# CPJKU/audio_sheet_retrieval

Hardware: AMD Instinct MI355X
Metric: snippet-pairs/sec embedded+ranked (32-d CCA) (higher is better)
Workload: dtype f32

## Files before the change

### audio_sheet_retrieval_amd/csrc/conv_wino_kernels.hip

```cpp
#include <hip/hip_runtime.h>
#include <stdint.h>
#include <stdlib.h>
#include <algorithm>
#include <type_traits>
#include <vector>
#include "asr_kernels.h"
#include "repack_elems.inl"
#include "wino_tile_order.h"
#include "wino_weight_layout.h"

#ifndef ASR_WINOG_NOCOPY
#define ASR_WINOG_NOCOPY 1
#endif

#ifndef ASR_WINOG_ABL
#define ASR_WINOG_ABL 0
#endif

namespace asr {

typedef float floatx4w __attribute__((ext_vector_type(4)));
typedef float float2w __attribute__((ext_vector_type(2)));

#ifndef ASR_WINO_ASMREAD
#define ASR_WINO_ASMREAD 1
#endif
#ifndef ASR_WINO_BUFDMA
#define ASR_WINO_BUFDMA 1
#endif

struct WinoArgs {
    const float *in;
    const float *wpk;
    const float *bnp;
    float *out;
    int N, H, W, OH, OW;
    int RY, RX;
    int MY, MX;
    int nmy, nmx;
    int tiles_y, tiles_x;
    int coutp;
    int C4P, RP;
    int total;
    int per;
    double *stats;
    BnBwdFuse bf;
    const void *raw;
    const float *w1;
    const float *bn1;
};

#ifndef ASR_WINO_PKADD
#define ASR_WINO_PKADD 1
#endif
__device__ __forceinline__ float ssub(float a, float b) {
    float r;
    asm("v_sub_f32 %0, %1, %2" : "=v"(r) : "v"(a), "v"(b));
    return r;
}
__device__ __forceinline__ float2w psub(float2w a, float2w b) {
    if (ASR_WINO_PKADD) return a - b;
    return float2w{ssub(a[0], b[0]), ssub(a[1], b[1])};
}
__device__ __forceinline__ floatx4w psub(floatx4w a, floatx4w b) {
    if (ASR_WINO_PKADD) return a - b;
    return floatx4w{ssub(a[0], b[0]), ssub(a[1], b[1]), ssub(a[2], b[2]), ssub(a[3], b[3])};
}
__device__ __forceinline__ float sadd(float a, float b) {
    float r;
    asm("v_add_f32 %0, %1, %2" : "=v"(r) : "v"(a), "v"(b));
    return r;
}
__device__ __forceinline__ float2w padd(float2w a, float2w b) {
    if (ASR_WINO_PKADD) return a + b;
    return float2w{sadd(a[0], b[0]), sadd(a[1], b[1])};
}
__device__ __forceinline__ floatx4w padd(floatx4w a, floatx4w b) {
    if (ASR_WINO_PKADD) return a + b;
    return floatx4w{sadd(a[0], b[0]), sadd(a[1], b[1]), sadd(a[2], b[2]), sadd(a[3], b[3])};
}

__device__ float4 g_wino_zero[4];

template <int NTV>
__device__ __forceinline__ void wino_stats_store(double *stats, int row, int cout, int col0, int lane,
                                                 const double (&s1)[NTV], const double (&s2)[NTV]) {
    const int g = lane >> 4, n = lane & 15;
#pragma unroll
    for (int nt = 0; nt < NTV; ++nt) {
        double a = s1[nt], b = s2[nt];
        a += __shfl_xor(a, 16); b += __shfl_xor(b, 16);
        a += __shfl_xor(a, 32); b += __shfl_xor(b, 32);
        const int ch = col0 + nt * 16 + n;
        if (g == 0 && ch < cout) {
            stats[((size_t)row * 2) * cout + ch] = a;
            stats[((size_t)row * 2 + 1) * cout + ch] = b;
        }
    }
}

__device__ __forceinline__ float elu_fastw(float y) { return y > 0.0f ? y : __expf(y) - 1.0f; }

template <int CIN, int COUT, bool POOL, int NTW, int KB, int WAVES, int MINW, int RMAX, bool RAW, int PW = 0,
          int IN_MODE = 0>
__global__ __launch_bounds__(64 * (WAVES + PW), MINW) void conv3x3_wino(WinoArgs a) {
    constexpr int KS = CIN / 4;
    constexpr int NB = CIN / 8;
    constexpr bool REM = (CIN % 8) != 0;
    constexpr int NCH = NB / KB;
    constexpr int WROW = NTW * 16;
    constexpr int WS = NTW == 2 ? 48 : WROW;
    constexpr int C4 = CIN / 4;
    constexpr int T = 64 * (WAVES + PW);
    static_assert(NB % KB == 0, "chunking must divide the channel blocks");
    static_assert(PW == 0 || (!RAW && NTW * 16 >= COUT), "producer builds: deterministic path, one n-group");
    extern __shared__ __align__(16) float lds[];
    const int tid = threadIdx.x, lane = tid & 63;
    const int wave = __builtin_amdgcn_readfirstlane(tid >> 6);
    const int LW = a.RX + 2, LH = a.RY + 2;
    constexpr int C4P = (C4 & 1) ? C4 : C4 + 1;
    constexpr int CSf = C4P * 4;
    const int RPf = a.RP * 4;
    const int buf_floats = (LH * RPf + 255) & ~255;
    float *w_lds = lds + 2 * buf_floats;
    const int ng = blockIdx.y;
    const int first = blockIdx.x * a.per;
    const int last = min(first + a.per, a.total);
    if (first >= last) return;

    for (int i = tid; i < 16 * KS * 4 * (WROW / 4); i += T) {
        const int row = i / (WROW / 4), q = i - row * (WROW / 4);
        const int col = ng * WROW + q * 4;
        float4 v = make_float4(0.f, 0.f, 0.f, 0.f);
        if (col < a.coutp) v = *reinterpret_cast<const float4 *>(a.wpk + (size_t)row * a.coutp + col);
        *reinterpret_cast<float4 *>(w_lds + row * WS + q * 4) = v;
    }
    constexpr int RMAXE = PW > 0 ? 1 : RMAX;
    int st_g[RMAXE], st_rc[RMAXE];
    if constexpr (PW == 0) {
#pragma unroll
        for (int k = 0; k < RMAX; ++k) {
            const int f = tid + k * T;
            const int r = f / a.RP;
            const int xs = f - r * a.RP - ((r >> 1) & 1);
            const int px = xs / C4P, c = xs - px * C4P;
            const bool real = r < LH && xs >= 0 && px < LW && c < C4;
#if ASR_WINO_BUFDMA
            st_g[k] = real ? (((r - 1) * a.W + (px - 1)) * CIN + c * 4) * 4 : (int)0x80000000;
#else
            st_g[k] = ((r - 1) * a.W + (px - 1)) * CIN + c * 4;
#endif
            st_rc[k] = real ? (r << 16) | px : -1;
        }
    }
    auto fetch = [&](int region, float *buf) {
        if constexpr (PW == 0) {
        const int tx = region % a.tiles_x;
        const int rest = region / a.tiles_x;
        const int ty = rest % a.tiles_y;
        const int img = rest / a.tiles_y;
        const int Y0 = ty * a.RY, X0 = tx * a.RX;
#if ASR_WINO_BUFDMA
        {
            typedef int int4v __attribute__((ext_vector_type(4)));
            const uint64_t ibase = reinterpret_cast<uint64_t>(a.in + (int64_t)img * a.H * a.W * CIN);
            int4v rsrc;
            rsrc.x = (int)(uint32_t)ibase;
            rsrc.y = (int)(uint32_t)(ibase >> 32);
            rsrc.z = a.H * a.W * CIN * 4;
            rsrc.w = 0x00020000;
            const int roff = (Y0 * a.W + X0) * CIN * 4;
            const unsigned lds0 = (unsigned)(uintptr_t)(__attribute__((address_space(3))) void *)buf;
            const bool xedge = X0 < 1 || X0 + LW - 1 > a.W;
            auto dma = [&](int k, int vo) {
                const unsigned m0v = lds0 + (unsigned)((k * T + wave * 64) * 16);
                asm volatile("s_mov_b32 m0, %2\n\ts_nop 0\n\tbuffer_load_dwordx4 %0, %1, 0 offen lds"
                             ::"v"(vo), "s"(rsrc), "s"(m0v)
                             : "memory", "m0");
            };
            if (!__builtin_amdgcn_readfirstlane((int)xedge)) {
#pragma unroll
                for (int k = 0; k < RMAX; ++k) {
                    if ((k * T + wave * 64) * 4 >= buf_floats) break;
                    dma(k, st_g[k] + roff);
                }
                return;
            }
#pragma unroll
            for (int k = 0; k < RMAX; ++k) {
                if ((k * T + wave * 64) * 4 >= buf_floats) break;
                const int x = X0 - 1 + (st_rc[k] & 0xffff);
                dma(k, (st_rc[k] >= 0 && (unsigned)x < (unsigned)a.W) ? st_g[k] + roff : (int)0x80000000);
            }
            return;
        }
#endif
        const float *gbase = a.in + (((int64_t)img * a.H + Y0) * a.W + X0) * CIN;
        if (!(ASR_WINOG_ABL & 512) && Y0 >= 1 && Y0 + LH - 1 <= a.H && X0 >= 1 && X0 + LW - 1 <= a.W) {
#pragma unroll
            for (int k = 0; k < RMAX; ++k) {
                if ((k * T + wave * 64) * 4 >= buf_floats) break;
                const float *src = st_rc[k] >= 0 ? gbase + st_g[k] : reinterpret_cast<const float *>(g_wino_zero);
                __builtin_amdgcn_global_load_lds((const __attribute__((address_space(1))) void *)src,
                                                 (__attribute__((address_space(3))) void *)(buf + (k * T + wave * 64) * 4),
                                                 16, 0, 0);
            }
            return;
        }
#pragma unroll
        for (int k = 0; k < RMAX; ++k) {
            if ((k * T + wave * 64) * 4 >= buf_floats) break;
            const int y = Y0 - 1 + (st_rc[k] >> 16), x = X0 - 1 + (st_rc[k] & 0xffff);
            const bool ok = st_rc[k] >= 0 && y >= 0 && y < a.H && x >= 0 && x < a.W;
            const float *src = ok ? gbase + st_g[k] : reinterpret_cast<const float *>(g_wino_zero);
            __builtin_amdgcn_global_load_lds((const __attribute__((address_space(1))) void *)src,
                                             (__attribute__((address_space(3))) void *)(buf + (k * T + wave * 64) * 4),
                                             16, 0, 0);
        }
        }
    };
    float *tab255 = w_lds + 16 * KS * 4 * WS;
    auto produce = [&](int region, float *buf) {
        if constexpr (PW > 0) {
        const int ptid = tid - 64 * WAVES;
        const int tx = region % a.tiles_x;
        const int rest = region / a.tiles_x;
        const int ty = rest % a.tiles_y;
        const int img = rest / a.tiles_y;
        const int Y0 = ty * a.RY, X0 = tx * a.RX;
        const size_t ioff = (size_t)img * a.H * a.W;
        const int npx = LH * LW;
        const float rcpLW = 1.0f / (float)LW;
        for (int f = ptid; f < npx; f += 64 * PW) {
            const int r = (int)(((float)f + 0.5f) * rcpLW), px = f - r * LW;
            const int y = Y0 - 1 + r, x = X0 - 1 + px;
            float *dst = buf + (r * a.RP + ((r >> 1) & 1) + px * C4P) * 4;
            if (y < 0 || y >= a.H || x < 0 || x >= a.W) {
#pragma unroll
                for (int c = 0; c < C4; ++c) *reinterpret_cast<float4 *>(dst + c * 4) = make_float4(0.f, 0.f, 0.f, 0.f);
                continue;
            }
            float v[9];
#pragma unroll
            for (int aa = 0; aa < 3; ++aa)
#pragma unroll
                for (int bb = 0; bb < 3; ++bb) {
                    const int yy = y - 1 + aa, xx = x - 1 + bb;
                    const bool ok = yy >= 0 && yy < a.H && xx >= 0 && xx < a.W;
                    const int yc = min(max(yy, 0), a.H - 1), xc = min(max(xx, 0), a.W - 1);
                    const size_t off = ioff + (size_t)yc * a.W + xc;
                    float val;
                    if (IN_MODE == 2) val = tab255[((const unsigned char *)a.raw)[off]];
                    else if (IN_MODE == 1) val = ((const float *)a.raw)[off] / 255.0f;
                    else val = ((const float *)a.raw)[off];
                    v[aa * 3 + bb] = ok ? val : 0.0f;
                }
            constexpr int C1P = (CIN + 15) / 16 * 16;
#pragma unroll 1
            for (int cg = 0; cg < C4; ++cg) {
                const float *wg = a.w1 + cg * 36;
                float res[4];
#pragma unroll
                for (int c = 0; c < 4; ++c) {
                    const int co = cg * 4 + c;
                    float acc = 0.0f;
#pragma unroll
                    for (int t = 0; t < 9; ++t) acc = fmaf(v[t], wg[c * 9 + t], acc);
                    res[c] = elu_fastw((acc - a.bn1[co]) * a.bn1[C1P + co] + a.bn1[2 * C1P + co]);
                }
                *reinterpret_cast<float4 *>(dst + cg * 4) = make_float4(res[0], res[1], res[2], res[3]);
            }
        }
        }
    };
    const bool producer = PW > 0 && wave >= WAVES;
    if constexpr (PW > 0) {
        if (IN_MODE == 2)
            for (int i = tid; i < 256; i += T) tab255[i] = (float)i / 255.0f;
        __syncthreads();
        if (producer) produce(first, lds);
    } else {
        fetch(first, lds);
#if ASR_WINO_BUFDMA
        asm volatile("s_waitcnt vmcnt(0)" ::: "memory");
#endif
    }
    __syncthreads();

    const int m = lane & 15, g = lane >> 4, n = lane & 15;
    const int tyy = m / a.MX, txx = m - tyy * a.MX;
    int a_row[4];
#pragma unroll
    for (int i = 0; i < 4; ++i)
        a_row[i] = (2 * tyy + i) * RPf + 2 * txx * CSf + ((tyy + (i >> 1)) & 1) * 4;
    const int a_pair = (g >> 1) * 4 + (g & 1) * 2;
    const int a_rem = NB * 8 + g;
    const float *w_lane = w_lds + g * WS + n;
    auto wq_off = [](int q) { return ((q / (16 * NTW)) * 16 + (q / NTW) % 16) * 4 * WS + (q % NTW) * 16; };
    int ey[4], ex[4], eoff[4];
#pragma unroll
    for (int r = 0; r < 4; ++r) {
        const int me = 4 * g + r;
        ey[r] = me / a.MX;
        ex[r] = me - ey[r] * a.MX;
        eoff[r] = (POOL ? ey[r] * a.OW + ex[r] : 2 * ey[r] * a.W + 2 * ex[r]) * COUT + ng * WROW + n;
    }
    float bmean[NTW], bscale[NTW], bbeta[NTW];
#pragma unroll
    for (int nt = 0; nt < NTW; ++nt) {
        const int ch = ng * WROW + nt * 16 + n;
        const bool ok = !RAW && ch < COUT;
        bmean[nt] = ok ? a.bnp[ch] : 0.f;
        bscale[nt] = ok ? a.bnp[a.coutp + ch] : 1.f;
        bbeta[nt] = ok ? a.bnp[2 * a.coutp + ch] : 0.f;
    }
    float bistd[NTW];
    const bool bnb = ASR_BNB_FUSE_BUILD && RAW && a.stats && a.bf.z != nullptr;
#pragma unroll
    for (int nt = 0; nt < NTW; ++nt) {
        const int ch = ng * WROW + nt * 16 + n;
        bistd[nt] = 0.f;
        if (bnb && ch < COUT) {
            bmean[nt] = a.bf.cst[ch]; bistd[nt] = a.bf.cst[COUT + ch];
            bscale[nt] = a.bf.cst[2 * COUT + ch]; bbeta[nt] = a.bf.cst[3 * COUT + ch];
        }
    }

    double st1[NTW], st2[NTW];
#pragma unroll
    for (int nt = 0; nt < NTW; ++nt) { st1[nt] = 0.0; st2[nt] = 0.0; }
    for (int region = first; region < last; ++region) {
    const float *in_lds = lds + ((region - first) & 1) * buf_floats;
    if (region + 1 < last && !(ASR_WINOG_ABL & 1)) {
        if constexpr (PW > 0) {
            if (producer) produce(region + 1, lds + ((region + 1 - first) & 1) * buf_floats);
        } else {
            fetch(region + 1, lds + ((region + 1 - first) & 1) * buf_floats);
        }
    }
    const int tx = region % a.tiles_x;
    const int rest = region / a.tiles_x;
    const int ty = rest % a.tiles_y;
    const int img = rest / a.tiles_y;
    const int Y0 = ty * a.RY, X0 = tx * a.RX;
    for (int mt = producer ? a.nmy * a.nmx : wave; mt < a.nmy * a.nmx; mt += WAVES) {
        const int mty = mt / a.nmx, mtx = mt - mty * a.nmx;
        const int oy = mty * a.MY * 2, ox = mtx * a.MX * 2;
        if (Y0 + oy >= a.H || X0 + ox >= a.W) continue;
        const float *ap = in_lds + oy * RPf + ox * CSf;
        floatx4w acc[16][NTW];
#pragma unroll
        for (int p = 0; p < 16; ++p)
#pragma unroll
            for (int nt = 0; nt < NTW; ++nt) acc[p][nt] = floatx4w{0.f, 0.f, 0.f, 0.f};

#pragma unroll
        for (int ch = 0; ch < NCH + (REM ? 1 : 0); ++ch) {
            if (ch < NCH) {
                float2w dp[4][4][KB];
#if ASR_WINO_ASMREAD
                if (ASR_WINOG_ABL & 32) {
#pragma unroll
                    for (int i = 0; i < 4; ++i)
#pragma unroll
                        for (int j = 0; j < 4; ++j)
#pragma unroll
                            for (int c = 0; c < KB; ++c) dp[i][j][c] = float2w{(float)i, (float)j};
                } else {
#pragma unroll
                    for (int i = 0; i < 4; ++i) {
                        const unsigned la = (unsigned)(uintptr_t)(const __attribute__((address_space(3))) void *)(ap + a_row[i] + a_pair);
#pragma unroll
                        for (int j = 0; j < 4; ++j)
#pragma unroll
                            for (int c = 0; c < KB; ++c)
                                asm volatile("ds_read_b64 %0, %1 offset:%2"
                                             : "=v"(dp[i][j][c])
                                             : "v"(la), "n"((j * CSf + (ch * KB + c) * 8) * 4));
                    }
#pragma unroll
                    for (int c = 0; c < KB; ++c)
                        asm volatile("s_waitcnt lgkmcnt(0)"
                                     : "+v"(dp[0][0][c]), "+v"(dp[0][1][c]), "+v"(dp[0][2][c]), "+v"(dp[0][3][c]),
                                       "+v"(dp[1][0][c]), "+v"(dp[1][1][c]), "+v"(dp[1][2][c]), "+v"(dp[1][3][c]),
                                       "+v"(dp[2][0][c]), "+v"(dp[2][1][c]), "+v"(dp[2][2][c]), "+v"(dp[2][3][c]),
                                       "+v"(dp[3][0][c]), "+v"(dp[3][1][c]), "+v"(dp[3][2][c]), "+v"(dp[3][3][c]));
                }
#else
#pragma unroll
                for (int i = 0; i < 4; ++i)
#pragma unroll
                    for (int j = 0; j < 4; ++j)
#pragma unroll
                        for (int c = 0; c < KB; ++c)
                            dp[i][j][c] = (ASR_WINOG_ABL & 32) ? float2w{(float)i, (float)j}
                                                               : *reinterpret_cast<const float2w *>(ap + a_row[i] + j * CSf + (ch * KB + c) * 8 + a_pair);
#endif
#pragma unroll
                for (int c = 0; c < KB; ++c) {
#pragma unroll
                    for (int j = 0; j < 4; ++j) {
                        const float2w d0 = dp[0][j][c], d1 = dp[1][j][c], d2 = dp[2][j][c], d3 = dp[3][j][c];
                        dp[0][j][c] = psub(d0, d2); dp[1][j][c] = padd(d1, d2); dp[2][j][c] = psub(d2, d1); dp[3][j][c] = psub(d1, d3);
                    }
#pragma unroll
                    for (int i = 0; i < 4; ++i) {
                        const float2w t0 = dp[i][0][c], t1 = dp[i][1][c], t2 = dp[i][2][c], t3 = dp[i][3][c];
                        dp[i][0][c] = psub(t0, t2); dp[i][1][c] = padd(t1, t2); dp[i][2][c] = psub(t2, t1); dp[i][3][c] = psub(t1, t3);
                    }
                }
                constexpr int WQ = 2 * KB * 16 * NTW, WD = 4 * NTW;
                const float *wk = w_lane + (ch * 2 * KB) * (16 * 4 * WS);
                float wv[WQ + WD];
#pragma unroll
                for (int q = 0; q < WD; ++q) wv[q] = wk[wq_off(q)];
#pragma unroll
                for (int q0 = 0; q0 < WQ; q0 += NTW) {
#pragma unroll
                    for (int q = q0; q < q0 + NTW; ++q)
                        wv[q + WD] = (ASR_WINOG_ABL & 16) ? wv[q] : (q + WD < WQ) ? wk[wq_off(q + WD)] : 0.f;
                    __builtin_amdgcn_sched_barrier(0);
#pragma unroll
                    for (int q = q0; q < q0 + NTW; ++q) {
                        const int p = (q / NTW) % 16, c = q / (16 * NTW), nt = q % NTW;
                        acc[p][nt] = __builtin_amdgcn_mfma_f32_16x16x4f32(dp[p >> 2][p & 3][c >> 1][c & 1], wv[q],
                                                                          acc[p][nt], 0, 0, 0);
                    }
                    __builtin_amdgcn_sched_barrier(0);
                }
            } else {
                float dsg[4][4];
#pragma unroll
                for (int i = 0; i < 4; ++i)
#pragma unroll
                    for (int j = 0; j < 4; ++j) dsg[i][j] = (ASR_WINOG_ABL & 32) ? (float)(i + j) : ap[a_row[i] + j * CSf + a_rem];
#pragma unroll
                for (int j = 0; j < 4; ++j) {
                    const float d0 = dsg[0][j], d1 = dsg[1][j], d2 = dsg[2][j], d3 = dsg[3][j];
                    dsg[0][j] = d0 - d2; dsg[1][j] = d1 + d2; dsg[2][j] = d2 - d1; dsg[3][j] = d1 - d3;
                }
#pragma unroll
                for (int i = 0; i < 4; ++i) {
                    const float t0 = dsg[i][0], t1 = dsg[i][1], t2 = dsg[i][2], t3 = dsg[i][3];
                    dsg[i][0] = t0 - t2; dsg[i][1] = t1 + t2; dsg[i][2] = t2 - t1; dsg[i][3] = t1 - t3;
                }
#pragma unroll
                for (int p = 0; p < 16; ++p)
#pragma unroll
                    for (int nt = 0; nt < NTW; ++nt)
                        acc[p][nt] = __builtin_amdgcn_mfma_f32_16x16x4f32(
                            dsg[p >> 2][p & 3], w_lane[((2 * NB * 16 + p) * 4) * WS + nt * 16], acc[p][nt], 0, 0, 0);
            }
        }

        const int py0 = Y0 + oy, px0 = X0 + ox;
        float *obase = POOL ? a.out + (((int64_t)img * a.OH + (py0 >> 1)) * a.OW + (px0 >> 1)) * COUT
                            : a.out + (((int64_t)img * a.H + py0) * a.W + px0) * COUT;
        const int ly = POOL ? a.OH - (py0 >> 1) : (a.H - py0 + 1) >> 1;
        const int lx = POOL ? a.OW - (px0 >> 1) : (a.W - px0 + 1) >> 1;
#pragma unroll
        for (int nt = 0; nt < NTW; ++nt) {
            if (ng * WROW + nt * 16 + n >= COUT) continue;
            floatx4w s0[4], s1[4];
#pragma unroll
            for (int nu = 0; nu < 4; ++nu) {
                s0[nu] = padd(padd(acc[nu][nt], acc[4 + nu][nt]), acc[8 + nu][nt]);
                s1[nu] = psub(psub(acc[4 + nu][nt], acc[8 + nu][nt]), acc[12 + nu][nt]);
            }
            const floatx4w y00 = padd(padd(s0[0], s0[1]), s0[2]), y01 = psub(psub(s0[1], s0[2]), s0[3]);
            const floatx4w y10 = padd(padd(s1[0], s1[1]), s1[2]), y11 = psub(psub(s1[1], s1[2]), s1[3]);
            const bool full = POOL ? (a.MY <= ly && a.MX <= lx) : (py0 + 2 * a.MY <= a.H && px0 + 2 * a.MX <= a.W);
            if (full && !(ASR_WINOG_ABL & 64)) {
#pragma unroll
                for (int r = 0; r < 4; ++r) {
                    float *o = obase + eoff[r] + nt * 16;
                    if (POOL) {
                        const float hi = fmaxf(fmaxf(y00[r], y01[r]), fmaxf(y10[r], y11[r]));
                        const float lo = fminf(fminf(y00[r], y01[r]), fminf(y10[r], y11[r]));
                        const float x = bscale[nt] >= 0.0f ? hi : lo;
                        o[0] = elu_fastw((x - bmean[nt]) * bscale[nt] + bbeta[nt]);
                    } else {
                        const int rstride = a.W * COUT;
                        const float v00 = RAW ? y00[r] : elu_fastw((y00[r] - bmean[nt]) * bscale[nt] + bbeta[nt]);
                        const float v01 = RAW ? y01[r] : elu_fastw((y01[r] - bmean[nt]) * bscale[nt] + bbeta[nt]);
                        const float v10 = RAW ? y10[r] : elu_fastw((y10[r] - bmean[nt]) * bscale[nt] + bbeta[nt]);
                        const float v11 = RAW ? y11[r] : elu_fastw((y11[r] - bmean[nt]) * bscale[nt] + bbeta[nt]);
                        o[0] = v00; o[COUT] = v01; o[rstride] = v10; o[rstride + COUT] = v11;
                        if (RAW && a.stats) {
                            if (bnb) {
                                const size_t e = (size_t)(o - a.out);
                                const float *zp = a.bf.z + e;
                                float t1 = 0.f, t2 = 0.f;
                                bnb_acc(v00, zp[0], bnb_mult(a.bf.tie, e), bmean[nt], bscale[nt], bbeta[nt], bistd[nt], t1, t2);
                                bnb_acc(v01, zp[COUT], bnb_mult(a.bf.tie, e + COUT), bmean[nt], bscale[nt], bbeta[nt], bistd[nt], t1, t2);
                                bnb_acc(v10, zp[rstride], bnb_mult(a.bf.tie, e + rstride), bmean[nt], bscale[nt], bbeta[nt], bistd[nt], t1, t2);
                                bnb_acc(v11, zp[rstride + COUT], bnb_mult(a.bf.tie, e + rstride + COUT), bmean[nt], bscale[nt], bbeta[nt], bistd[nt], t1, t2);
                                st1[nt] += (double)t1; st2[nt] += (double)t2;
                            } else {
                            st1[nt] += (double)((v00 + v01) + (v10 + v11));
                            st2[nt] += (double)((v00 * v00 + v01 * v01) + (v10 * v10 + v11 * v11));
                            }
                        }
                    }
                }
                continue;
            }
#pragma unroll
            for (int r = 0; r < 4; ++r) {
                if (ey[r] >= ly || ex[r] >= lx) continue;
                float *o = obase + eoff[r] + nt * 16;
                if (ASR_WINOG_ABL & 64) {
                    asm volatile("" ::"v"(y00[r]), "v"(y01[r]), "v"(y10[r]), "v"(y11[r]));
                    continue;
                }
                if (POOL) {
                    const float hi = fmaxf(fmaxf(y00[r], y01[r]), fmaxf(y10[r], y11[r]));
                    const float lo = fminf(fminf(y00[r], y01[r]), fminf(y10[r], y11[r]));
                    const float x = bscale[nt] >= 0.0f ? hi : lo;
                    o[0] = elu_fastw((x - bmean[nt]) * bscale[nt] + bbeta[nt]);
                } else {
                    const bool y1 = 2 * ey[r] + 1 < a.H - py0, x1 = 2 * ex[r] + 1 < a.W - px0;
                    const int rstride = a.W * COUT;
                    const float v00 = RAW ? y00[r] : elu_fastw((y00[r] - bmean[nt]) * bscale[nt] + bbeta[nt]);
                    const float v01 = RAW ? y01[r] : elu_fastw((y01[r] - bmean[nt]) * bscale[nt] + bbeta[nt]);
                    const float v10 = RAW ? y10[r] : elu_fastw((y10[r] - bmean[nt]) * bscale[nt] + bbeta[nt]);
                    const float v11 = RAW ? y11[r] : elu_fastw((y11[r] - bmean[nt]) * bscale[nt] + bbeta[nt]);
                    o[0] = v00;
                    if (x1) o[COUT] = v01;
                    if (y1) o[rstride] = v10;
                    if (y1 && x1) o[rstride + COUT] = v11;
                    if (RAW && a.stats) {
                        if (bnb) {
                            const size_t e = (size_t)(o - a.out);
                            const float *zp = a.bf.z + e;
                            float t1 = 0.f, t2 = 0.f;
                            bnb_acc(v00, zp[0], bnb_mult(a.bf.tie, e), bmean[nt], bscale[nt], bbeta[nt], bistd[nt], t1, t2);
                            if (x1) bnb_acc(v01, zp[COUT], bnb_mult(a.bf.tie, e + COUT), bmean[nt], bscale[nt], bbeta[nt], bistd[nt], t1, t2);
                            if (y1) bnb_acc(v10, zp[rstride], bnb_mult(a.bf.tie, e + rstride), bmean[nt], bscale[nt], bbeta[nt], bistd[nt], t1, t2);
                            if (y1 && x1) bnb_acc(v11, zp[rstride + COUT], bnb_mult(a.bf.tie, e + rstride + COUT), bmean[nt], bscale[nt], bbeta[nt], bistd[nt], t1, t2);
                            st1[nt] += (double)t1; st2[nt] += (double)t2;
                        } else {
                        const float w01 = x1 ? v01 : 0.f, w10 = y1 ? v10 : 0.f, w11 = (y1 && x1) ? v11 : 0.f;
                        st1[nt] += (double)((v00 + w01) + (w10 + w11));
                        st2[nt] += (double)((v00 * v00 + w01 * w01) + (w10 * w10 + w11 * w11));
                        }
                    }
                }
            }
        }
    }
#if ASR_WINO_BUFDMA
    if constexpr (PW == 0) asm volatile("s_waitcnt vmcnt(0)" ::: "memory");
#endif
    __syncthreads();
    }
    if (RAW && a.stats)
        wino_stats_store<NTW>(a.stats, (int)blockIdx.x * WAVES + wave, COUT, ng * WROW, lane, st1, st2);
}

struct WinoGArgs {
    const float *in, *wpk, *bnp;
    float *out;
    int N, H, W, OH, OW;
    int coutp;
    int tiles;
    int total;
    WinoTileOrder ord;
    double *stats;
    BnBwdFuse bf;
};

template <int CIN, int COUT, bool POOL, int NT, int WAVES, int MINW, bool RAW>
__global__ __launch_bounds__(64 * WAVES, MINW) void conv3x3_winog(WinoGArgs a) {
    constexpr int KS = CIN / 4, NB = CIN / 8, WROW = NT * 16, T = 64 * WAVES;
    constexpr bool DENSE = wino_w_dense(CIN, NT);
    constexpr int KF = wino_w_kstep_floats(CIN, NT);
    constexpr int WD = 4 * NT;
    constexpr int WQ = 32 * NT;
    constexpr bool REM = (CIN % 8) != 0;
    constexpr bool PIPE = (MINW == 1);
    constexpr bool EARLY = !PIPE && !REM;
    static_assert(CIN % 4 == 0, "k-steps of 4 channels");
    extern __shared__ __align__(16) float w_lds[];
    const int tid = threadIdx.x, lane = tid & 63;
    const int wave = __builtin_amdgcn_readfirstlane(tid >> 6);
    const int ng = blockIdx.y;
    if constexpr (DENSE) {
#pragma unroll 1
        for (int i = tid; i < 16 * CIN * 4; i += T) {
            const int row = i >> 2, n4 = (i & 3) * 4;
            float v[NT][4];
#pragma unroll
            for (int nt = 0; nt < NT; ++nt) {
                const int col = ng * WROW + nt * 16 + n4;
                float4 x = make_float4(0.f, 0.f, 0.f, 0.f);
                if (col < a.coutp) x = *reinterpret_cast<const float4 *>(a.wpk + (size_t)row * a.coutp + col);
                v[nt][0] = x.x; v[nt][1] = x.y; v[nt][2] = x.z; v[nt][3] = x.w;
            }
#pragma unroll
            for (int e = 0; e < 4; ++e)
#pragma unroll
                for (int nt = 0; nt < NT; ++nt) w_lds[wino_w_stage_off(CIN, NT, row, nt * 16 + n4 + e)] = v[nt][e];
        }
    } else {
// ... 356 lines not shown
                    pend[nt][r][0] = elu_fastw((x - bmean[nt]) * bscale[nt] + bbeta[nt]);
                } else {
                    pend[nt][r][0] = RAW ? y00[r] : elu_fastw((y00[r] - bmean[nt]) * bscale[nt] + bbeta[nt]);
                    pend[nt][r][PV - 3] = RAW ? y01[r] : elu_fastw((y01[r] - bmean[nt]) * bscale[nt] + bbeta[nt]);
                    pend[nt][r][PV - 2] = RAW ? y10[r] : elu_fastw((y10[r] - bmean[nt]) * bscale[nt] + bbeta[nt]);
                    pend[nt][r][PV - 1] = RAW ? y11[r] : elu_fastw((y11[r] - bmean[nt]) * bscale[nt] + bbeta[nt]);
                    if (RAW && a.stats) {
                        const int f = pend_flags[r];
                        if (bnb) {
                            if ((f & 1) && ng * WROW + nt * 16 + n < COUT) {
                                const size_t e = (size_t)pend_off[r] + ng * WROW + nt * 16 + n;
                                const float *zp = a.bf.z + e;
                                const int rstride = a.W * COUT;
                                float t1 = 0.f, t2 = 0.f;
                                bnb_acc(y00[r], zp[0], bnb_mult(a.bf.tie, e), bmean[nt], bscale[nt], bbeta[nt], bistd[nt], t1, t2);
                                if ((f & 3) == 3) bnb_acc(y01[r], zp[COUT], bnb_mult(a.bf.tie, e + COUT), bmean[nt], bscale[nt], bbeta[nt], bistd[nt], t1, t2);
                                if ((f & 5) == 5) bnb_acc(y10[r], zp[rstride], bnb_mult(a.bf.tie, e + rstride), bmean[nt], bscale[nt], bbeta[nt], bistd[nt], t1, t2);
                                if ((f & 7) == 7) bnb_acc(y11[r], zp[rstride + COUT], bnb_mult(a.bf.tie, e + rstride + COUT), bmean[nt], bscale[nt], bbeta[nt], bistd[nt], t1, t2);
                                gst1[nt] += (double)t1; gst2[nt] += (double)t2;
                            }
                        } else {
                        const float w00 = (f & 1) ? y00[r] : 0.f, w01 = ((f & 3) == 3) ? y01[r] : 0.f;
                        const float w10 = ((f & 5) == 5) ? y10[r] : 0.f, w11 = ((f & 7) == 7) ? y11[r] : 0.f;
                        gst1[nt] += (double)((w00 + w01) + (w10 + w11));
                        gst2[nt] += (double)((w00 * w00 + w01 * w01) + (w10 * w10 + w11 * w11));
                        }
                    }
                }
            }
        }
        if (PIPE) {
            have_pend = true;
        } else {
            flush();
            if (!EARLY && mt + mt_stride < mt_end) {
                setup(mt + mt_stride);
                load_first();
                if (REM) load_rem();
            }
        }
    }
    if (PIPE) flush();
    if (RAW && a.stats)
        wino_stats_store<NT>(a.stats, (int)blockIdx.x * WAVES + wave, COUT, ng * WROW, lane, gst1, gst2);
}

__global__ void wino_pack_kernel(const float *W, int cin, int cout, int dgrad, float *wpk) {
    const int idx = blockIdx.x * blockDim.x + threadIdx.x;
    if (idx >= wino_pack_count(cin, cout, dgrad)) return;
    wino_pack_elem(idx, W, cin, cout, dgrad, wpk);
}

size_t wino_wpack_floats(int cin, int cout) { return (size_t)16 * cin * ((cout + 15) / 16 * 16); }

hipError_t launch_wino_pack(hipStream_t s, const float *W, int cin, int cout, float *wpk, int dgrad) {
    const int kdim = dgrad ? cout : cin, ndim = dgrad ? cin : cout;
    const int total = kdim * ((ndim + 15) / 16 * 16);
    hipLaunchKernelGGL(wino_pack_kernel, dim3((total + 255) / 256), dim3(256), 0, s, W, cin, cout, dgrad, wpk);
    return hipGetLastError();
}

struct WinoVariant {
    int cin, cout, pool, ntw, kb, waves, minw, rmax, raw;
    void (*kernel)(WinoArgs);
    const char *symbol;
    int pw, in_mode;
};
#define ASR_BOOLSTRW_0 "false"
#define ASR_BOOLSTRW_1 "true"
#define ASR_WINO(CIN, COUT, POOL, NTW, KB, WAVES, MINW, RMAX)                                                     \
    { CIN, COUT, POOL, NTW, KB, WAVES, MINW, RMAX, 0,                                                             \
      conv3x3_wino<CIN, COUT, (POOL != 0), NTW, KB, WAVES, MINW, RMAX, false>,                                    \
      "void asr::conv3x3_wino<" #CIN ", " #COUT ", " ASR_BOOLSTRW_##POOL ", " #NTW ", " #KB ", " #WAVES ", " #MINW \
      ", " #RMAX ", false, 0, 0>(asr::WinoArgs)" }
#define ASR_WINOR(CIN, COUT, NTW, KB, WAVES, MINW, RMAX)                                                          \
    { CIN, COUT, 0, NTW, KB, WAVES, MINW, RMAX, 1,                                                                \
      conv3x3_wino<CIN, COUT, false, NTW, KB, WAVES, MINW, RMAX, true>,                                           \
      "void asr::conv3x3_wino<" #CIN ", " #COUT ", false, " #NTW ", " #KB ", " #WAVES ", " #MINW                  \
      ", " #RMAX ", true, 0, 0>(asr::WinoArgs)" }
#define ASR_WINOF1(CIN, COUT, WAVES, MINW, PW, MODE)                                                              \
    { CIN, COUT, 1, 1, 1, WAVES, MINW, 1, 0,                                                                      \
      conv3x3_wino<CIN, COUT, true, 1, 1, WAVES, MINW, 1, false, PW, MODE>,                                       \
      "void asr::conv3x3_wino<" #CIN ", " #COUT ", true, 1, 1, " #WAVES ", " #MINW ", 1, false, " #PW ", " #MODE  \
      ">(asr::WinoArgs)", PW, MODE }
#define ASR_WINOF(CIN, COUT, WAVES, MINW, PW)                                                                     \
    ASR_WINOF1(CIN, COUT, WAVES, MINW, PW, 0), ASR_WINOF1(CIN, COUT, WAVES, MINW, PW, 1),                         \
        ASR_WINOF1(CIN, COUT, WAVES, MINW, PW, 2)
static const WinoVariant g_wino[] = {
    ASR_WINO(12, 12, 1, 1, 1, 4, 3, 8),
    ASR_WINO(12, 12, 1, 1, 1, 8, 3, 6),
    ASR_WINO(12, 24, 0, 2, 1, 4, 2, 8),
    ASR_WINO(12, 24, 0, 2, 1, 8, 2, 6),
    ASR_WINO(12, 24, 0, 1, 1, 4, 3, 8),
    ASR_WINO(24, 24, 1, 2, 1, 4, 2, 8),
    ASR_WINO(24, 24, 1, 2, 1, 8, 2, 6),
    ASR_WINO(24, 24, 1, 1, 3, 4, 2, 10),
    ASR_WINO(24, 24, 1, 1, 1, 8, 2, 6),
    ASR_WINO(24, 48, 0, 1, 3, 4, 2, 10),
    ASR_WINO(24, 48, 0, 1, 1, 8, 2, 8),
    ASR_WINO(24, 48, 0, 2, 1, 8, 2, 6),
    ASR_WINO(48, 48, 1, 1, 2, 4, 2, 12),
    ASR_WINO(48, 48, 1, 1, 2, 8, 2, 10),
    ASR_WINO(48, 48, 1, 1, 1, 8, 2, 8),
    ASR_WINO(48, 48, 0, 1, 2, 4, 2, 12),
    ASR_WINO(48, 48, 0, 1, 2, 8, 2, 10),
    ASR_WINO(48, 48, 0, 1, 1, 8, 2, 8),
    ASR_WINOR(12, 12, 1, 1, 8, 3, 6),
    ASR_WINOR(12, 24, 2, 1, 8, 2, 6),
    ASR_WINOR(12, 12, 1, 1, 4, 3, 8),
    ASR_WINOR(12, 24, 2, 1, 4, 2, 8),
    ASR_WINOR(12, 24, 1, 1, 4, 3, 8),
    ASR_WINOF(12, 12, 4, 4, 4), ASR_WINOF(12, 12, 4, 3, 2), ASR_WINOF(12, 12, 8, 3, 4), ASR_WINOF(12, 12, 8, 4, 8),
    ASR_WINOF(12, 12, 4, 3, 4),
};
static const int g_num_wino = (int)(sizeof(g_wino) / sizeof(g_wino[0]));

static int wino_lds_layout(int cin, int LW, int MY, int MX, int *c4p_out, int *rp_out) {
    const int c4 = cin / 4;
    const int c4p = (c4 & 1) ? c4 : c4 + 1;
    int best_rp = 0, best = 1 << 30;
    for (int extra = 1; extra <= 8; ++extra) {
        const int rp = LW * c4p + extra;
        int worst = 0;
        for (int half = 0; half < 2; ++half)
            for (int i = 0; i < 4; ++i) {
                int seen[64][32], nseen[64] = {0};
                int cycles = 1;
                for (int l = 0; l < 32; ++l) {
                    const int lane = half * 32 + l;
                    const int m = lane & 15, g = lane >> 4;
                    const int tyy = m / MX, txx = m % MX;
                    const int fl = ((2 * tyy + i) * rp + 2 * txx * c4p + ((tyy + (i >> 1)) & 1)) * 4 + (g >> 1) * 4 + (g & 1) * 2;
                    for (int w = 0; w < 2; ++w) {
                        const int bank = (fl + w) & 63;
                        bool dup = false;
                        for (int q = 0; q < nseen[bank]; ++q) dup = dup || seen[bank][q] == fl + w;
                        if (!dup) seen[bank][nseen[bank]++] = fl + w;
                        cycles = std::max(cycles, nseen[bank]);
                    }
                }
                worst = std::max(worst, cycles);
            }
        if (worst < best) { best = worst; best_rp = rp; }
    }
    *c4p_out = c4p;
    *rp_out = best_rp;
    return best;
}

static void enumerate_wino(int vi, int H, int W, int lds_budget, std::vector<ConvPlan> &out) {
    const WinoVariant &v = g_wino[vi];
    const int nt = (v.cout + 15) / 16;
    const int ngroups = (nt + v.ntw - 1) / v.ntw;
    const int w_bytes = 16 * v.cin * (v.ntw == 2 ? 48 : v.ntw * 16) * 4;
    static const int shapes[4][2] = {{2, 8}, {4, 4}, {8, 2}, {16, 1}};
    const int ty_img = (H + 1) / 2, tx_img = (W + 1) / 2;
    for (const auto &sh : shapes) {
        const int MY = sh[0], MX = sh[1];
        const int max_my = (ty_img + MY - 1) / MY, max_mx = (tx_img + MX - 1) / MX;
        for (int nmy = 1; nmy <= max_my; ++nmy) {
            for (int nmx = 1; nmx <= max_mx; ++nmx) {
                const int RY = nmy * MY * 2, RX = nmx * MX * 2;
                int c4p = 0, rp = 0;
                const int rd_cycles = wino_lds_layout(v.cin, RX + 2, MY, MX, &c4p, &rp);
                const int patch_f4 = (RY + 2) * rp;
                const int lds = 2 * ((patch_f4 * 16 + 1023) & ~1023) + w_bytes + (v.pw ? 1024 : 0);
                if (lds > lds_budget) continue;
                if (!v.pw && patch_f4 > v.rmax * 64 * v.waves) continue;
                const int n_mt = nmy * nmx;
                if (n_mt > 16 * v.waves) continue;
                const int tiles_y = (H + RY - 1) / RY, tiles_x = (W + RX - 1) / RX;
                const double per_wave = (double)((n_mt + v.waves - 1) / v.waves);
                const double mfma = 16.0 * (v.cin / 4) * v.ntw * 32.0;
                const double valu = (16.0 * (v.cin / 4) + 110.0 * v.ntw) * 4.0 + (rd_cycles - 1) * 8.0 * v.cin;
                double stage = (double)v.rmax * 16.0 * 4.0;
                if (v.pw) {
                    const double prod = std::ceil((RY + 2.0) * (RX + 2.0) / (64.0 * v.pw)) * 330.0 * 4.0;
                    const double cons = (16.0 * (v.cin / 4) * v.ntw * 32.0 + (16.0 * (v.cin / 4) + 110.0 * v.ntw) * 4.0) *
                                        (double)((n_mt + v.waves - 1) / v.waves);
                    stage = prod > cons ? prod - cons : 0.0;
                }
                ConvPlan bp{};
                bp.cost = ((mfma + valu) * per_wave + stage + 800.0) * tiles_y * tiles_x * ngroups;
                bp.TH = RY; bp.TW = RX; bp.NI = MY;
                bp.tiles_y = tiles_y; bp.tiles_x = tiles_x;
                bp.lds_bytes = lds;
                bp.tile_floats = nmy * 1000 + nmx;
                bp.c4p = c4p; bp.rp = rp;
                bp.cin = v.cin; bp.cout = v.cout; bp.pool = v.pool;
                bp.H = H; bp.W = W;
                bp.OH = v.pool ? H / 2 : H;
                bp.OW = v.pool ? W / 2 : W;
                bp.threads = 64 * (v.waves + v.pw);
                bp.variant = 3000 + vi;
                bp.symbol = v.symbol;
                bp.fuse1 = v.pw ? 1 : 0;
                out.push_back(bp);
            }
        }
    }
    std::sort(out.begin(), out.end(), [](const ConvPlan &x, const ConvPlan &y) { return x.cost < y.cost; });
}

static void finish_wino(ConvPlan &bp) {
    const WinoVariant &v = g_wino[bp.variant - 3000];
    for (int mode = 0; mode < (v.pw ? 3 : 1); ++mode)
        (void)hipFuncSetAttribute(reinterpret_cast<const void *>(g_wino[bp.variant - 3000 + mode].kernel),
                                  hipFuncAttributeMaxDynamicSharedMemorySize, 160 * 1024);
    int nb = 0;
    if (hipOccupancyMaxActiveBlocksPerMultiprocessor(&nb, reinterpret_cast<const void *>(v.kernel), bp.threads,
                                                     (size_t)bp.lds_bytes) != hipSuccess || nb < 1) {
        (void)hipGetLastError();
        nb = std::max(1, std::min(4, (160 * 1024) / std::max(1, bp.lds_bytes)));
    }
    bp.blocks_per_cu = std::min(nb, 8);
}

struct WinoGVariant {
    int cin, cout, pool, nt, waves, minw, raw;
    void (*kernel)(WinoGArgs);
    const char *symbol;
};
#define ASR_WINOG(CIN, COUT, POOL, NT, WAVES, MINW)                                                               \
    { CIN, COUT, POOL, NT, WAVES, MINW, 0, conv3x3_winog<CIN, COUT, (POOL != 0), NT, WAVES, MINW, false>,         \
      "void asr::conv3x3_winog<" #CIN ", " #COUT ", " ASR_BOOLSTRW_##POOL ", " #NT ", " #WAVES ", " #MINW         \
      ", false>(asr::WinoGArgs)" }
#define ASR_WINOGR(CIN, COUT, NT, WAVES, MINW)                                                                    \
    { CIN, COUT, 0, NT, WAVES, MINW, 1, conv3x3_winog<CIN, COUT, false, NT, WAVES, MINW, true>,                   \
      "void asr::conv3x3_winog<" #CIN ", " #COUT ", false, " #NT ", " #WAVES ", " #MINW ", true>(asr::WinoGArgs)" }
static const WinoGVariant g_winog[] = {
    ASR_WINOG(12, 12, 1, 1, 4, 2), ASR_WINOG(12, 12, 1, 1, 8, 2), ASR_WINOG(12, 24, 0, 2, 4, 2), ASR_WINOG(12, 24, 0, 2, 4, 1),
    ASR_WINOG(24, 24, 1, 2, 4, 1), ASR_WINOG(24, 24, 1, 2, 4, 2), ASR_WINOG(24, 24, 1, 2, 8, 2),
    ASR_WINOG(24, 48, 0, 3, 4, 1),
    ASR_WINOG(48, 48, 1, 3, 4, 1), ASR_WINOG(48, 48, 0, 3, 4, 1),
    ASR_WINOG(48, 96, 0, 3, 4, 1), ASR_WINOG(96, 96, 1, 1, 8, 2), ASR_WINOG(96, 96, 0, 1, 8, 2),
    ASR_WINOG(96, 96, 1, 1, 4, 2), ASR_WINOG(96, 96, 0, 1, 4, 2),
    ASR_WINOGR(24, 24, 2, 4, 2), ASR_WINOGR(24, 48, 3, 4, 1), ASR_WINOGR(48, 48, 3, 4, 1),
    ASR_WINOGR(24, 12, 1, 4, 2), ASR_WINOGR(48, 24, 2, 4, 2),
    ASR_WINOGR(24, 24, 2, 8, 2), ASR_WINOGR(24, 24, 2, 4, 1), ASR_WINOGR(48, 24, 2, 8, 2), ASR_WINOGR(48, 24, 2, 4, 1),
    ASR_WINOGR(24, 12, 1, 8, 2),
    ASR_WINOGR(48, 96, 3, 4, 1), ASR_WINOGR(96, 96, 1, 8, 2), ASR_WINOGR(96, 48, 1, 8, 2),
};
static const int g_num_winog = (int)(sizeof(g_winog) / sizeof(g_winog[0]));

static void candidates_winog(int cin, int cout, int pool, int H, int W, std::vector<ConvPlan> *out, int raw = 0) {
    for (int vi = 0; vi < g_num_winog; ++vi) {
        const WinoGVariant &v = g_winog[vi];
        if (v.cin != cin || v.cout != cout || v.pool != pool || v.raw != raw) continue;
        const int lds = wino_w_lds_floats(cin, v.nt) * 4;
        if (lds > 160 * 1024) continue;
        (void)hipFuncSetAttribute(reinterpret_cast<const void *>(v.kernel), hipFuncAttributeMaxDynamicSharedMemorySize,
                                  160 * 1024);
        int nb = 0;
        if (hipOccupancyMaxActiveBlocksPerMultiprocessor(&nb, reinterpret_cast<const void *>(v.kernel), 64 * v.waves,
                                                         (size_t)lds) != hipSuccess || nb < 1) {
            (void)hipGetLastError();
            nb = 1;
        }
        ConvPlan bp{};
        bp.cin = cin; bp.cout = cout; bp.pool = pool;
        bp.H = H; bp.W = W; bp.OH = pool ? H / 2 : H; bp.OW = pool ? W / 2 : W;
        bp.TH = 2; bp.TW = 32; bp.NI = 16;
        bp.tiles_y = pool ? bp.OH : (H + 1) / 2; bp.tiles_x = pool ? bp.OW : (W + 1) / 2;
        bp.threads = 64 * v.waves;
        bp.lds_bytes = lds;
        bp.blocks_per_cu = std::min(nb, 4);
        bp.cost = (double)bp.tiles_y * bp.tiles_x / 16.0 * ((cout + 15) / 16 + v.nt - 1) / v.nt *
                  (16.0 * (cin / 4) * v.nt * 32.0 + 1500.0);
        bp.variant = 3500 + vi;
        bp.symbol = v.symbol;
        out->push_back(bp);
        if (!raw)
            for (int S : {1}) {
                bp.TH = S;
                bp.cost *= 1.01;
                out->push_back(bp);
            }
    }
}

void conv_candidates_wino(int cin, int cout, int pool, int H, int W, int max_count, std::vector<ConvPlan> *out) {
    static const int use = getenv("ASR_CONV_WINO") ? atoi(getenv("ASR_CONV_WINO")) : 1;
    if (!use) return;
    candidates_winog(cin, cout, pool, H, W, out);
    for (int vi = 0; vi < g_num_wino; ++vi) {
        const WinoVariant &v = g_wino[vi];
        if (v.cin != cin || v.cout != cout || v.pool != pool || v.raw || v.pw) continue;
        for (int budget : {52 * 1024, 78 * 1024, 158 * 1024}) {
            std::vector<ConvPlan> c;
            enumerate_wino(vi, H, W, budget, c);
            int taken = 0;
            for (auto &cand : c) {
                bool dup = false;
                for (auto &o : *out)
                    if (o.variant == cand.variant && o.TH == cand.TH && o.TW == cand.TW && o.NI == cand.NI) dup = true;
                if (dup) continue;
                finish_wino(cand);
                out->push_back(cand);
                if (++taken >= max_count) break;
            }
        }
    }
}

void conv_candidates_wino_fused(int cin, int cout, int pool, int H, int W, int max_count, std::vector<ConvPlan> *out) {
    static const int use = getenv("ASR_CONV_WINO") ? atoi(getenv("ASR_CONV_WINO")) : 1;
    if (!use) return;
// ... 142 lines not shown
```

Measured before the change: 310,800.

## Pack Winograd weights densely in LDS for paired float2 reads

```diff
diff --git a/audio_sheet_retrieval_amd/csrc/conv_wino_kernels.hip b/audio_sheet_retrieval_amd/csrc/conv_wino_kernels.hip
--- a/audio_sheet_retrieval_amd/csrc/conv_wino_kernels.hip
+++ b/audio_sheet_retrieval_amd/csrc/conv_wino_kernels.hip
@@ -8,6 +8,7 @@
 #include "repack_elems.inl"
 #include "wino_tile_order.h"
 #include "wino_weight_layout.h"
+#include "wino_lds_weight_layout.h"
 
 #ifndef ASR_WINOG_NOCOPY
 #define ASR_WINOG_NOCOPY 1
@@ -109,7 +110,11 @@
     constexpr bool REM = (CIN % 8) != 0;
     constexpr int NCH = NB / KB;
     constexpr int WROW = NTW * 16;
-    constexpr int WS = NTW == 2 ? 48 : WROW;
+    constexpr bool DENSE = wino_lw_dense(NTW, PW);
+    constexpr int WS = wino_lw_row_stride(NTW);
+    constexpr int WLDS = wino_lw_lds_floats(CIN, NTW, DENSE);
+    constexpr int RPK = wino_lw_reads_per_kstep(NTW);
+    constexpr int WDR = NTW == 2 ? 4 : 2;
     constexpr int C4 = CIN / 4;
     constexpr int T = 64 * (WAVES + PW);
     static_assert(NB % KB == 0, "chunking must divide the channel blocks");
@@ -128,12 +133,20 @@
     const int last = min(first + a.per, a.total);
     if (first >= last) return;
 
+#pragma unroll 1
     for (int i = tid; i < 16 * KS * 4 * (WROW / 4); i += T) {
         const int row = i / (WROW / 4), q = i - row * (WROW / 4);
         const int col = ng * WROW + q * 4;
         float4 v = make_float4(0.f, 0.f, 0.f, 0.f);
         if (col < a.coutp) v = *reinterpret_cast<const float4 *>(a.wpk + (size_t)row * a.coutp + col);
-        *reinterpret_cast<float4 *>(w_lds + row * WS + q * 4) = v;
+        if constexpr (DENSE) {
+            w_lds[wino_lw_stage_off(NTW, true, row, q * 4)] = v.x;
+            w_lds[wino_lw_stage_off(NTW, true, row, q * 4 + 1)] = v.y;
+            w_lds[wino_lw_stage_off(NTW, true, row, q * 4 + 2)] = v.z;
+            w_lds[wino_lw_stage_off(NTW, true, row, q * 4 + 3)] = v.w;
+        } else {
+            *reinterpret_cast<float4 *>(w_lds + wino_lw_stage_off(NTW, false, row, q * 4)) = v;
+        }
     }
     constexpr int RMAXE = PW > 0 ? 1 : RMAX;
     int st_g[RMAXE], st_rc[RMAXE];
@@ -219,7 +232,7 @@
         }
         }
     };
-    float *tab255 = w_lds + 16 * KS * 4 * WS;
+    float *tab255 = w_lds + WLDS;
     auto produce = [&](int region, float *buf) {
         if constexpr (PW > 0) {
         const int ptid = tid - 64 * WAVES;
@@ -295,8 +308,8 @@
         a_row[i] = (2 * tyy + i) * RPf + 2 * txx * CSf + ((tyy + (i >> 1)) & 1) * 4;
     const int a_pair = (g >> 1) * 4 + (g & 1) * 2;
     const int a_rem = NB * 8 + g;
-    const float *w_lane = w_lds + g * WS + n;
-    auto wq_off = [](int q) { return ((q / (16 * NTW)) * 16 + (q / NTW) % 16) * 4 * WS + (q % NTW) * 16; };
+    const float *w_lane = w_lds + wino_lw_lane_off(NTW, DENSE, g, n);
+    auto wq_off = [](int q) { return wino_lw_rowmajor_off(NTW, q / (16 * NTW), (q / NTW) % 16, q % NTW); };
     int ey[4], ex[4], eoff[4];
 #pragma unroll
     for (int r = 0; r < 4; ++r) {
@@ -409,6 +422,29 @@
                         dp[i][0][c] = psub(t0, t2); dp[i][1][c] = padd(t1, t2); dp[i][2][c] = psub(t2, t1); dp[i][3][c] = psub(t1, t3);
                     }
                 }
+                if constexpr (DENSE) {
+                    constexpr int NR = 2 * KB * RPK;
+                    const int r0 = ch * NR;
+                    float2w wv[NR + WDR];
+#pragma unroll
+                    for (int r = 0; r < WDR; ++r)
+                        wv[r] = *reinterpret_cast<const float2w *>(w_lane + wino_lw_read_off(r0 + r));
+#pragma unroll
+                    for (int r = 0; r < NR; ++r) {
+                        wv[r + WDR] = (ASR_WINOG_ABL & 16) ? wv[r]
+                                      : (r + WDR < NR) ? *reinterpret_cast<const float2w *>(w_lane + wino_lw_read_off(r0 + r + WDR))
+                                                       : float2w{0.f, 0.f};
+                        __builtin_amdgcn_sched_barrier(0);
+#pragma unroll
+                        for (int e = 0; e < 2; ++e) {
+                            const int c = wino_lw_read_kstep(NTW, r), p = wino_lw_read_pos(NTW, r, e);
+                            const int nt = wino_lw_read_ntile(NTW, e);
+                            acc[p][nt] = __builtin_amdgcn_mfma_f32_16x16x4f32(dp[p >> 2][p & 3][c >> 1][c & 1], wv[r][e],
+                                                                              acc[p][nt], 0, 0, 0);
+                        }
+                        __builtin_amdgcn_sched_barrier(0);
+                    }
+                } else {
                 constexpr int WQ = 2 * KB * 16 * NTW, WD = 4 * NTW;
                 const float *wk = w_lane + (ch * 2 * KB) * (16 * 4 * WS);
                 float wv[WQ + WD];
@@ -428,6 +464,7 @@
                     }
                     __builtin_amdgcn_sched_barrier(0);
                 }
+                }
             } else {
                 float dsg[4][4];
 #pragma unroll
@@ -444,12 +481,32 @@
                     const float t0 = dsg[i][0], t1 = dsg[i][1], t2 = dsg[i][2], t3 = dsg[i][3];
                     dsg[i][0] = t0 - t2; dsg[i][1] = t1 + t2; dsg[i][2] = t2 - t1; dsg[i][3] = t1 - t3;
                 }
-#pragma unroll
-                for (int p = 0; p < 16; ++p)
-#pragma unroll
-                    for (int nt = 0; nt < NTW; ++nt)
-                        acc[p][nt] = __builtin_amdgcn_mfma_f32_16x16x4f32(
-                            dsg[p >> 2][p & 3], w_lane[((2 * NB * 16 + p) * 4) * WS + nt * 16], acc[p][nt], 0, 0, 0);
+                if constexpr (DENSE) {
+                    constexpr int r0 = 2 * NB * RPK;
+                    float2w wv[RPK + WDR];
+#pragma unroll
+                    for (int r = 0; r < WDR; ++r)
+                        wv[r] = *reinterpret_cast<const float2w *>(w_lane + wino_lw_read_off(r0 + r));
+#pragma unroll
+                    for (int r = 0; r < RPK; ++r) {
+                        wv[r + WDR] = (r + WDR < RPK) ? *reinterpret_cast<const float2w *>(w_lane + wino_lw_read_off(r0 + r + WDR))
+                                                      : float2w{0.f, 0.f};
+                        __builtin_amdgcn_sched_barrier(0);
+#pragma unroll
+                        for (int e = 0; e < 2; ++e) {
+                            const int p = wino_lw_read_pos(NTW, r, e), nt = wino_lw_read_ntile(NTW, e);
+                            acc[p][nt] = __builtin_amdgcn_mfma_f32_16x16x4f32(dsg[p >> 2][p & 3], wv[r][e], acc[p][nt], 0, 0, 0);
+                        }
+                        __builtin_amdgcn_sched_barrier(0);
+                    }
+                } else {
+#pragma unroll
+                    for (int p = 0; p < 16; ++p)
+#pragma unroll
+                        for (int nt = 0; nt < NTW; ++nt)
+                            acc[p][nt] = __builtin_amdgcn_mfma_f32_16x16x4f32(
+                                dsg[p >> 2][p & 3], w_lane[wino_lw_rowmajor_off(NTW, 2 * NB, p, nt)], acc[p][nt], 0, 0, 0);
+                }
             }
         }
 
@@ -1112,7 +1169,7 @@
     const WinoVariant &v = g_wino[vi];
     const int nt = (v.cout + 15) / 16;
     const int ngroups = (nt + v.ntw - 1) / v.ntw;
-    const int w_bytes = 16 * v.cin * (v.ntw == 2 ? 48 : v.ntw * 16) * 4;
+    const int w_bytes = wino_lw_lds_floats(v.cin, v.ntw, wino_lw_dense(v.ntw, v.pw)) * 4;
     static const int shapes[4][2] = {{2, 8}, {4, 4}, {8, 2}, {16, 1}};
     const int ty_img = (H + 1) / 2, tx_img = (W + 1) / 2;
     for (const auto &sh : shapes) {
diff --git a/audio_sheet_retrieval_amd/csrc/wino_lds_weight_layout.h b/audio_sheet_retrieval_amd/csrc/wino_lds_weight_layout.h
--- /dev/null
+++ b/audio_sheet_retrieval_amd/csrc/wino_lds_weight_layout.h
@@ -0,0 +1,44 @@
+#pragma once
+
+#if defined(__HIPCC__)
+#define ASR_LWLAY_HD __host__ __device__ __forceinline__ constexpr
+#else
+#define ASR_LWLAY_HD inline constexpr
+#endif
+
+#ifndef ASR_WINO_DENSEW
+#define ASR_WINO_DENSEW 1
+#endif
+
+namespace asr {
+
+ASR_LWLAY_HD bool wino_lw_dense(int ntw, int pw) { return ASR_WINO_DENSEW && pw == 0 && (ntw == 1 || ntw == 2); }
+
+ASR_LWLAY_HD int wino_lw_row_stride(int ntw) { return ntw == 2 ? 48 : 16 * ntw; }
+
+ASR_LWLAY_HD int wino_lw_lds_floats(int cin, int ntw, bool dense) {
+    return 16 * cin * (dense ? 16 * ntw : wino_lw_row_stride(ntw));
+}
+
+ASR_LWLAY_HD int wino_lw_stage_off(int ntw, bool dense, int row, int col) {
+    if (!dense) return row * wino_lw_row_stride(ntw) + col;
+    if (ntw == 2) return (row * 16 + (col & 15)) * 2 + (col >> 4);
+    const int ks = row >> 6, p = (row >> 2) & 15, g = row & 3;
+    return (((ks * 8 + (p >> 1)) * 4 + g) * 16 + col) * 2 + (p & 1);
+}
+
+ASR_LWLAY_HD int wino_lw_lane_off(int ntw, bool dense, int g, int n) {
+    return dense ? (g * 16 + n) * 2 : g * wino_lw_row_stride(ntw) + n;
+}
+
+ASR_LWLAY_HD int wino_lw_reads_per_kstep(int ntw) { return 8 * ntw; }
+ASR_LWLAY_HD int wino_lw_read_off(int r) { return r * 128; }
+ASR_LWLAY_HD int wino_lw_read_kstep(int ntw, int r) { return r / (8 * ntw); }
+ASR_LWLAY_HD int wino_lw_read_pos(int ntw, int r, int e) { return ntw == 2 ? r % 16 : 2 * (r % 8) + e; }
+ASR_LWLAY_HD int wino_lw_read_ntile(int ntw, int e) { return ntw == 2 ? e : 0; }
+
+ASR_LWLAY_HD int wino_lw_rowmajor_off(int ntw, int ks, int p, int nt) {
+    return (ks * 16 + p) * 4 * wino_lw_row_stride(ntw) + nt * 16;
+}
+
+}
```

After: 314,600, median of 6. 1.01x the previous value.
